# eso28599/resnmtf

Measured on AMD Instinct MI355X. Metric: multiplicative-update iters/sec (all views), higher is better.
Workload: dtype f32

## Files before the change

### resnmtf_amd/csrc/resnmtf_hip.hip

```cpp
#include <hip/hip_runtime.h>
#include <hip/hip_ext.h>

#include <algorithm>
#include <chrono>
#include <cmath>
#include <cstdlib>
#include <cstdio>
#include <cstring>
#include <random>
#include <string>
#include <thread>
#include <type_traits>
#include <vector>

#include "resnmtf_hip.h"
#include "resnmtf_kernels.hip.inc"
#include "resnmtf_sparse.hip.inc"
#include "resnmtf_jsd.hip.inc"
#include "resnmtf_group.hip.inc"
#include "resnmtf_bisil.hip.inc"
#include "resnmtf_split_tu.h"
#ifdef RESNMTF_SPLIT_TU
#define RESNMTF_EXTERN(NW, UNR, XG, MA) extern template __global__ void pass_kernel<1, NW, UNR, XG, MA, 0>(PassArgs, KKFArgs, KKSArgs);
RESNMTF_PASS_K16_LIST(RESNMTF_EXTERN)
#undef RESNMTF_EXTERN
#endif

namespace {

std::string g_create_error;

inline int round_up(int x, int a) { return (x + a - 1) / a * a; }
inline int ceil_div(int x, int a) { return (x + a - 1) / a; }

struct SharedMap {
  bool set = false;
  int count = -1;
  int* dev = nullptr;
  bool identity = false;
};

struct ViewState {
  int n = 0, m = 0, k = 0, KP = 16, NT = 1;
  bool owned = true, has_x = false, has_factors = false;
  int empty_rows = 0, empty_cols = 0;
  std::vector<unsigned char> empty_mask;
  unsigned char* ref_cl = nullptr;
  int ref_k = 0;
  int n_pad = 0, m_pad = 0;
  size_t ldx = 0, ldxt = 0;
  size_t x32_floats = 0, xt32_floats = 0;
  bool half = false, u16 = false;
  bool half_capable = false;
  double x_relerr = 0.0;
  _Float16 *X16 = nullptr, *Xt16 = nullptr;
  size_t ld16x = 0, ld16xt = 0, x16_halves = 0, xt16_halves = 0;
  float xscale = 1.f;
  float *X32 = nullptr, *Xt32 = nullptr;
  double* xnorm2 = nullptr;
  double *F = nullptr, *G = nullptr, *S = nullptr, *lambda = nullptr, *mu = nullptr;
  float *F32 = nullptr, *G32 = nullptr, *T32 = nullptr;
  unsigned short *Fk = nullptr, *Gk = nullptr;
  int nsplit_xg = 1, rps_xg = 64, nw_xg = 4, nsaux_xg = 1, rpsaux_xg = 64;
  int nsplit_xtf = 1, rps_xtf = 64, nw_xtf = 4, nsaux_xtf = 1, rpsaux_xtf = 64;
  int tw_xg = 8, tw_xtf = 8;
  float *Pxg = nullptr, *Pxtf = nullptr, *Paux_xg = nullptr, *Paux_xtf = nullptr;
  int *cnt_xg = nullptr, *cnt_xtf = nullptr;
  int* fuse_cnt = nullptr;
  int rpbF = 16, nblkF = 1, rpbG = 16, nblkG = 1;
  void* fblk = nullptr;
  size_t fblk_bytes = 0;
  float* Usum = nullptr;
  bool f_replica = false;
  void* gblk = nullptr; size_t gblk_bytes = 0;
  float* Tsum = nullptr;
  bool g_replica = false;
  double* sblk = nullptr;
  bool pp_xg = false, pp_xtf = false;
  int kk_mode = 0;
  double *partF = nullptr, *partG = nullptr;
  double *FtF = nullptr, *FtFS = nullptr, *cF = nullptr;
  double *Ma_F = nullptr, *Md_F = nullptr, *Ma_G = nullptr, *Md_G = nullptr;
  std::vector<SharedMap> row_map, col_map;
  UpdateArgs argF{}, argG{};
  KKFArgs argKF{};
  KKSArgs argKS{};
  PassArgs passXG{}, passXtF{};
  bool sparse = false;
  long long nnz_cap = 0, nnz = 0;
  long long *cp = nullptr, *rp = nullptr;
  int *ri = nullptr, *ci = nullptr;
  float *vcsc = nullptr, *vcsr = nullptr;
  int *blk_xg = nullptr, *blk_xtf = nullptr;
  int nblk_xg = 0, nblk_xtf = 0;
};

}

struct resnmtf_handle {
  int V = 0;
  std::vector<ViewState> views;
  resnmtf_options opt{};
  hipStream_t stream = nullptr;
  bool own_stream = false;
  std::vector<double> phi, xi, psi;
  SweepCtl* ctl = nullptr;
  double* err = nullptr;
// ... 101 lines not shown
auto pick_int(int x, F&& f) {
  if constexpr (sizeof...(Vs) == 0) return f(std::integral_constant<int, V0>{});
  else return x == V0 ? f(std::integral_constant<int, V0>{}) : pick_int<Vs...>(x, f);
}
template <class F>
auto pick_kp(int KP, F&& f) { return pick_int<16, 32, 48, 64>(KP, f); }
template <class F>
auto pick_bools(F&& f) { return f(); }
template <class F, class... Bs>
auto pick_bools(F&& f, bool b, Bs... bs) {
  return b ? pick_bools([&](auto... cs) { return f(std::true_type{}, cs...); }, bs...)
           : pick_bools([&](auto... cs) { return f(std::false_type{}, cs...); }, bs...);
}
constexpr int kKPs[] = {16, 32, 48, 64};
constexpr bool kBools[] = {false, true};

void free_view(ViewState& v) {
  if (v.fblk) { v.fblk = nullptr; v.Usum = nullptr; v.Ma_F = nullptr; v.Md_F = nullptr; v.lambda = nullptr; }
  if (v.gblk) { v.gblk = nullptr; v.Tsum = nullptr; v.Ma_G = nullptr; v.Md_G = nullptr; v.mu = nullptr; }
  v.sblk = nullptr;
  void* ptrs[] = {v.fuse_cnt, v.Fk, v.Gk, v.X16, v.Xt16, v.X32, v.Xt32, v.xnorm2, v.F, v.G, v.S, v.lambda, v.mu, v.F32, v.G32, v.T32, v.Pxg, v.Pxtf,
                  v.Paux_xg, v.Paux_xtf, v.cnt_xg, v.cnt_xtf, v.partF, v.partG, v.FtF, v.FtFS, v.cF, v.Ma_F, v.Md_F, v.Ma_G, v.Md_G, v.ref_cl,
                  v.cp, v.rp, v.ri, v.ci, v.vcsc, v.vcsr, v.blk_xg, v.blk_xtf};
  for (void* p : ptrs)
    if (p) (void)hipFree(p);
  for (auto& mp : v.row_map)
    if (mp.dev) (void)hipFree(mp.dev);
  for (auto& mp : v.col_map)
    if (mp.dev) (void)hipFree(mp.dev);
}

int check_view(resnmtf_handle* h, int v) {
  if (!h) return RESNMTF_ERR_INVALID;
  if (v < 0 || v >= h->V) return h->fail(RESNMTF_ERR_INVALID, "view index out of range");
  return RESNMTF_OK;
}

void to_row_major(const double* src, int rows, int cols, std::vector<double>& dst) {
  dst.resize((size_t)rows * cols);
  for (int j = 0; j < cols; ++j)
    for (int i = 0; i < rows; ++i) dst[(size_t)i * cols + j] = src[(size_t)j * rows + i];
}
void to_col_major(const std::vector<double>& src, int rows, int cols, double* dst) {
  for (int j = 0; j < cols; ++j)
    for (int i = 0; i < rows; ++i) dst[(size_t)j * rows + i] = src[(size_t)i * cols + j];
}

size_t update_smem_bytes(int KP) {
  const int UT = update_threads(KP), RG = UT / KP;
  const int P16 = (KP % 32 == 0) ? KP + 16 : KP + 32;
  return sizeof(double) * ((size_t)2 * KP * P16 + 2 * (size_t)RG * (KP + 2) + (size_t)RG * KP + 2 * UT + 2 * (size_t)RG * P16);
}
size_t kk_smem_bytes(int KP, int NW) { return sizeof(double) * ((size_t)4 * KP * KP + 3 * 64 * (size_t)NW); }
size_t pass_smem_bytes(int KP, int NW) {
  const size_t tile_form = std::max(sizeof(float) * (size_t)std::max(NW / 2, 1) * 64 * KP, kk_smem_bytes(KP, NW));
  return KP > 16 ? std::max(tile_form, wide_smem_bytes(KP / 16)) : tile_form;
}
constexpr int kMaxLds = 160 * 1024;

int max_pass_waves(int NT) { return NT <= 1 ? 16 : 8; }
int pass_blocks_per_cu(int NT, int nw) { return pass_min_blocks(NT, nw); }

using PassFn = void (*)(PassArgs, KKFArgs, KKSArgs);
using FusedFn = void (*)(PassArgs, KKFArgs, KKSArgs, UpdateArgs, FuseArgs);
using SpmmFn = void (*)(SpmmArgs, KKFArgs, KKSArgs);
template <int NVB> using WideFn = void (*)(WideChainArgs<NVB>);

struct PassK16Form { int nw, unroll; bool xg, mode_a; PassFn fn; };
const PassK16Form kPassK16[] = {
#define RESNMTF_FORM(NW, UNR, XG, MA) {NW, UNR, XG, MA, &pass_kernel<1, NW, UNR, XG, MA, 0>},
    RESNMTF_PASS_K16_LIST(RESNMTF_FORM)
#undef RESNMTF_FORM
};
PassFn select_pass(int NT, int nw, int unroll, bool xg, bool mode_a, bool wide) {
  if (NT <= 1) {
    for (const PassK16Form& f : kPassK16)
      if (!wide && f.nw == nw && f.unroll == unroll && f.xg == xg && f.mode_a == mode_a) return f.fn;
    return nullptr;
  }
  if (nw != 8 || unroll != 4) return nullptr;
  return pick_int<2, 3, 4>(NT, [&](auto nt) { return pick_bools([](auto x, auto m, auto w) {
    return &pass_kernel<decltype(nt)::value, 8, 4, decltype(x)::value, decltype(m)::value, (decltype(w)::value ? 3 : 0)>; }, xg, mode_a, wide); });
}
PassFn select_pass_half(int unroll, bool xg, bool u16) {
  return pick_int<2, 3, 6, 4>(unroll, [&](auto un) { return pick_bools([](auto x, auto u) { return &pass_half_kernel<decltype(un)::value, decltype(x)::value, decltype(u)::value>; }, xg, u16); });
}
FusedFn select_pass_fused(int unroll, bool xg, bool pre) {
  return pick_int<4, 8>(unroll, [&](auto un) { return pick_bools([](auto x, auto p) { return &pass_fused_kernel<decltype(un)::value, decltype(x)::value, decltype(p)::value>; }, xg, pre); });
}
SpmmFn select_spmm(int KP, bool xg) {
  return pick_kp(KP, [&](auto kp) { return pick_bools([](auto x) { return &spmm_kernel<decltype(kp)::value, decltype(x)::value>; }, xg); });
}
constexpr int kCoupleBuckets[] = {0, 4, 8, RESNMTF_MAX_COUPLE};
int couple_bucket(const UpdateArgs& a) { return !a.restricted ? 0 : a.n_couple <= 4 ? 4 : a.n_couple <= 8 ? 8 : RESNMTF_MAX_COUPLE; }
auto select_update(int KP, bool g, int bucket, bool emit) {
  return pick_kp(KP, [&](auto kp) { return pick_int<0, 4, 8, RESNMTF_MAX_COUPLE>(bucket, [&](auto nc) {
    return pick_bools([](auto G, auto E) { return &factor_update_kernel<decltype(kp)::value, decltype(G)::value, decltype(nc)::value, decltype(E)::value>; }, g, emit);
  }); });
}
template <int NVB>
auto select_f_chain(bool g, bool one_slab) { return g ? &f_chain_kernel<NVB, 1, true> : one_slab ? &f_chain_kernel<NVB, 1> : &f_chain_kernel<NVB, 4>; }
template <int NVB>
WideFn<NVB> select_wide_chain(int KP, bool g, bool sliced) {
  return pick_kp(KP, [&](auto kp) { return pick_bools([](auto G, auto S) -> WideFn<NVB> {
    constexpr int K = decltype(kp)::value;
    if constexpr (decltype(S)::value) return &wide_chain_kernel<K, decltype(G)::value, NVB, true>;
    else if constexpr (K >= 32) return &wide_chain_kernel<K, decltype(G)::value, NVB>;
    else return nullptr;
  }, g, sliced); });
}
template <int NVB>
auto select_slice_chain(int KP, bool g) {
  return pick_kp(KP, [&](auto kp) { return pick_bools([](auto G) { return &slice_chain_kernel<decltype(kp)::value, decltype(G)::value, NVB>; }, g); });
}
template <int NVB>
auto select_slice_products(int KP) { return pick_kp(KP, [](auto kp) { return &slice_products_kernel<decltype(kp)::value, NVB>; }); }
template <int NVB>
auto select_slice_walk(int KP) { return pick_kp(KP, [](auto kp) { return &slice_walk_kernel<decltype(kp)::value, NVB, 4>; }); }
auto select_slice_unpack(int KP) { return pick_kp(KP, [](auto kp) { return &slice_unpack_kernel<decltype(kp)::value>; }); }
constexpr int kSChainViews[] = {4, 8, RESNMTF_MAX_COUPLE + 1};
auto select_s_chain(int KP, int n_views) {
  const int nvb = n_views <= 4 ? 4 : n_views <= 8 ? 8 : RESNMTF_MAX_COUPLE + 1;
  return pick_kp(KP, [&](auto kp) { return pick_int<4, 8, RESNMTF_MAX_COUPLE + 1>(nvb, [](auto nv) { return &s_chain_kernel<decltype(kp)::value, decltype(nv)::value>; }); });
}

hipError_t set_all_attrs() {
  hipError_t e = hipSuccess;
  auto lds = [&](auto* fn, size_t bytes) {
    if (e == hipSuccess && fn) e = hipFuncSetAttribute(reinterpret_cast<const void*>(fn), hipFuncAttributeMaxDynamicSharedMemorySize, (int)bytes);
  };
  for (const PassK16Form& f : kPassK16) lds(f.fn, kMaxLds);
  for (bool xg : kBools)
    for (bool b : kBools) {
      for (int NT : {2, 3, 4}) { lds(select_pass(NT, 8, 4, xg, b, false), kMaxLds); lds(select_pass(NT, 8, 4, xg, b, true), kMaxLds); }
      for (int unroll : {4, 8}) lds(select_pass_fused(unroll, xg, b), kMaxLds);
    }
  for (int KP : kKPs) {
    for (bool g : kBools) {
      for (int bucket : kCoupleBuckets) { lds(select_update(KP, g, bucket, false), update_smem_bytes(KP)); lds(select_update(KP, g, bucket, true), update_smem_bytes(KP)); }
      for (bool sliced : kBools) { lds(select_wide_chain<4>(KP, g, sliced), wide_chain_smem_bytes(KP)); lds(select_wide_chain<8>(KP, g, sliced), wide_chain_smem_bytes(KP)); }
      lds(select_slice_chain<4>(KP, g), slice_chain_smem_bytes(KP, 4)); lds(select_slice_chain<8>(KP, g), slice_chain_smem_bytes(KP, 8));
      lds(select_spmm(KP, g), kk_smem_bytes(KP, 8));
    }
    for (int views : kSChainViews) lds(select_s_chain(KP, views), kMaxLds - 4096);
  }
  for (bool g : kBools)
    for (bool one_slab : kBools) { lds(select_f_chain<2>(g, one_slab), f_chain_smem_bytes<2>()); lds(select_f_chain<4>(g, one_slab), f_chain_smem_bytes<4>()); lds(select_f_chain<8>(g, one_slab), f_chain_smem_bytes<8>()); }
  return e;
}

SpmmArgs spmm_args(const ViewState& v, bool xg) {
  SpmmArgs a{};
  if (xg) { a.ptr = v.rp; a.idx = v.ci; a.val = v.vcsr; a.blk = v.blk_xg; a.nblk = v.nblk_xg; a.nsplit = v.nsplit_xg; a.B = v.G32; a.P = v.Pxg; a.cols_pad = v.n_pad; }
  else { a.ptr = v.cp; a.idx = v.ri; a.val = v.vcsc; a.blk = v.blk_xtf; a.nblk = v.nblk_xtf; a.nsplit = v.nsplit_xtf; a.B = v.F32; a.P = v.Pxtf; a.cols_pad = v.m_pad; }
  a.ldb = v.KP;
  return a;
}
dim3 spmm_grid(const SpmmArgs& a) { return dim3((a.kk_block0 ? 1 : 0) + ceil_div(a.nblk * a.nsplit, 8)); }
size_t spmm_smem(const SpmmArgs& a, int KP) { return a.kk_block0 && !a.no_kk ? kk_smem_bytes(KP, 8) : 0; }
void launch_spmm(resnmtf_handle* h, const SpmmArgs& a, int KP, bool xg, const KKFArgs& kf, const KKSArgs& ks) {
  launch(h, -1, select_spmm(KP, xg), spmm_grid(a), dim3(512), spmm_smem(a, KP), a, kf, ks);
}

struct PassLaunch {
  int image = 0;
  bool mode_a = true;
  bool fused = false;
  bool wide = false;
  bool xcd_order = false;
  bool short_last = false;
  bool pingpong = false;
  int waves = 8;
  int unroll = 0;
  int tiles_per_wg = 1;
  int lead_blocks = 1, main_blocks = 0;
  dim3 grid, block;
  size_t smem = 0;
  PassFn kern = nullptr;
  FusedFn kern_fused = nullptr;
  SpmmFn kern_spmm = nullptr;
};
PassLaunch resolve_pass(const resnmtf_handle* h, const ViewState& v, bool xg, bool fuse_update = false) {
  PassLaunch L;
  if (v.sparse) {
    SpmmArgs a = spmm_args(v, xg);
    a.kk_block0 = 1;
    L.image = 1;
    L.main_blocks = ceil_div(a.nblk * a.nsplit, 8);
    L.grid = spmm_grid(a); L.block = dim3(512);
    L.smem = spmm_smem(a, v.KP);
    L.kern_spmm = select_spmm(v.KP, xg);
    return L;
  }
  const int nw = xg ? v.nw_xg : v.nw_xtf, nsplit = xg ? v.nsplit_xg : v.nsplit_xtf, rps = xg ? v.rps_xg : v.rps_xtf;
  const int rows_pad = xg ? v.m_pad : v.n_pad, ntiles = (xg ? v.n_pad : v.m_pad) / 64;
  L.image = v.half ? (v.u16 ? 3 : 2) : 0;
  L.mode_a = v.kk_mode == 0;
  L.waves = nw;
  L.wide = v.NT >= 2 && h->opt.bf16_split != 2;
  L.xcd_order = L.wide && h->opt.xcd_order;
  L.short_last = nsplit > 1 && rows_pad - (nsplit - 1) * rps < rps;
  L.tiles_per_wg = L.wide ? (xg ? v.tw_xg : v.tw_xtf) : 1;
  L.main_blocks = ceil_div(ntiles, L.tiles_per_wg) * nsplit;
  L.lead_blocks = L.mode_a ? 1 : (xg ? 3 * v.nsaux_xg : 2 * v.nsaux_xtf);
  L.grid = dim3(L.lead_blocks + L.main_blocks); L.block = dim3(64 * nw);
  L.smem = std::min<size_t>(pass_smem_bytes(v.KP, nw) + (size_t)h->opt.pass_lds_pad_kb * 1024, kMaxLds);
  const bool pp = xg ? v.pp_xg : v.pp_xtf;
  if (fuse_update) {
    L.fused = true;
    L.pingpong = pp;
    L.unroll = pp ? 4 : 8;
    L.smem = std::min<size_t>(std::max(L.smem, update_smem_bytes(16)), kMaxLds);
    L.kern_fused = select_pass_fused(L.unroll, xg, h->opt.fuse_updates == 1);
  } else if (v.half) {
    const int hu = h->opt.half_unroll;
    L.unroll = (hu == 2 || hu == 3 || hu == 4 || hu == 6) ? hu : (v.u16 ? 2 : 4);
    L.kern = select_pass_half(L.unroll, xg, v.u16);
  } else {
    L.pingpong = v.NT == 1 && nw == 8 && pp;
    L.unroll = v.NT >= 2 ? 4 : (nw == 8 ? (pp ? 4 : RESNMTF_K16_UNROLL) : 8);
    L.kern = select_pass(v.NT, nw, L.unroll, xg, L.mode_a, L.wide);
  }
  return L;
}
bool can_fuse_update(const resnmtf_handle* h, const ViewState& v, int kind) {
  if (h->opt.fuse_updates == 0 || v.NT != 1 || !v.fuse_cnt) return false;
  const PassLaunch L = resolve_pass(h, v, kind != 0);
  if (L.image != 0 || !L.mode_a || L.waves != 8) return false;
  const UpdateArgs& u = kind == 0 ? v.argF : v.argG;
  const int nblk = kind == 0 ? v.nblkF : v.nblkG;
  return !u.restricted && nblk <= L.main_blocks && nblk <= h->n_cu;
}
void launch_pass(resnmtf_handle* h, const ViewState& v, bool xg, int mode, double tol, bool check_done, bool fuse_update = false) {
  const PassLaunch L = resolve_pass(h, v, xg, fuse_update);
  const int kind = xg ? RESNMTF_TIMED_XG : RESNMTF_TIMED_XTF;
  KKFArgs kf = v.argKF;
  KKSArgs ks = v.argKS;
  ks.mode = mode; ks.tol = tol;
  if (L.kern_spmm) {
    SpmmArgs a = spmm_args(v, xg);
    a.kk_block0 = 1; a.no_kk = 0; a.ctl = h->ctl; a.check_done = check_done ? 1 : 0;
    launch(h, kind, L.kern_spmm, L.grid, L.block, L.smem, a, kf, ks);
    return;
  }
  PassArgs a = xg ? v.passXG : v.passXtF;
  a.check_done = check_done ? 1 : 0;
  a.kk_block0 = L.mode_a ? 1 : 0;
  a.fuse_zero = (a.kk_block0 && v.fuse_cnt && !v.half) ? v.fuse_cnt + (xg ? 0 : 2) : nullptr;
  if (!a.kk_block0) { kf.part = nullptr; ks.part = nullptr; }
  a.xcd_n = 0;
  if (L.xcd_order) {
    const int n_map = L.short_last ? (a.nsplit - 1) * a.ntg : L.main_blocks;
    int cnt[8] = {0, 0, 0, 0, 0, 0, 0, 0};
    for (int x = 0; x < 8; ++x) a.xcd_first[x] = -1;
    for (int b = 0; b < n_map; ++b) {
      const int x = (L.lead_blocks + b) & 7;
      if (a.xcd_first[x] < 0) a.xcd_first[x] = L.lead_blocks + b;
      ++cnt[x];
    }
    int off = 0;
    for (int x = 0; x < 8; ++x) { a.xcd_off[x] = off; off += cnt[x]; if (a.xcd_first[x] < 0) a.xcd_first[x] = 0; }
    a.xcd_n = n_map;
  }
  if (L.fused) {
    UpdateArgs u = xg ? v.argG : v.argF;
    u.check_done = 0; u.gram_only = 0;
    FuseArgs fz{};
    fz.cnt_own = v.fuse_cnt + (xg ? 2 : 0);
    { static const int nap = std::getenv("RESNMTF_FUSE_NAP") ? std::atoi(std::getenv("RESNMTF_FUSE_NAP")) : 2; fz.nap = nap; }
    fz.n_upd = xg ? v.nblkG : v.nblkF; fz.err = h->fuse_err_dev;
    launch(h, kind, L.kern_fused, L.grid, L.block, L.smem, a, kf, ks, u, fz);
    return;
  }
  if (L.image >= 2) a.out_scale = v.u16 ? 1.f / v.xscale : 1.f / (v.xscale * RESNMTF_B16_SCALE);
  launch(h, kind, L.kern, L.grid, L.block, L.smem, a, kf, ks);
}

void launch_pass_plain(resnmtf_handle* h, PassArgs a, int NT, bool xg) {
  a.kk_block0 = 1; a.no_kk = 1; a.check_done = 0;
  const dim3 grid(1 + a.ntiles * a.nsplit), block(64 * 8);
  const size_t smem = std::min<size_t>(pass_smem_bytes(16 * NT, 8), kMaxLds);
  launch(h, -1, select_pass(NT, 8, NT <= 1 ? RESNMTF_K16_UNROLL : 4, xg, true, false), grid, block, smem, a, KKFArgs{}, KKSArgs{});
}

template <int NVB>
ChainArgs<NVB> narrow_chain(const ChainArgs<8>& c) {
  ChainArgs<NVB> a{};
  a.len = c.len; a.k = c.k; a.n_views = c.n_views; a.rows_per_block = c.rows_per_block;
  a.n_emit = c.n_emit; a.restricted = c.restricted; a.ctl = c.ctl; a.check_done = c.check_done; a.pstride = c.pstride;
  a.kpack32 = c.kpack32;
  for (int e = 0; e < 4; ++e) { a.W32e[e] = c.W32e[e]; a.parte[e] = c.parte[e]; a.T32e[e] = c.T32e[e]; }
  for (int v = 0; v < NVB; ++v) {
    a.emit_slot[v] = c.emit_slot[v];
    a.W[v] = c.W[v]; a.U[v] = c.U[v]; a.nsplit[v] = c.nsplit[v]; a.Ma[v] = c.Ma[v]; a.Md[v] = c.Md[v]; a.lm[v] = c.lm[v];
    a.sigma[v] = c.sigma[v]; a.n_other[v] = c.n_other[v]; a.cmask[v] = c.cmask[v];
    for (int w = 0; w < NVB; ++w) a.weight[v][w] = c.weight[v][w];
  }
  return a;
}

void launch_update(resnmtf_handle* h, const ViewState& v, int kind, bool check_done) {
  UpdateArgs a = kind == 0 ? v.argF : v.argG;
  a.check_done = check_done ? 1 : 0;
  a.gram_only = kind == 2 ? 1 : 0;
  if (kind == 2) { a.restricted = 0; a.n_couple = 0; }
  const int nblk = kind == 0 ? v.nblkF : v.nblkG;
  launch(h, -1, select_update(v.KP, kind != 0, couple_bucket(a), v.kk_mode == 0), dim3(nblk), dim3(update_threads(v.KP)), update_smem_bytes(v.KP), a);
}

template <int NVB>
WideChainArgs<NVB> narrow_wchain(const WideChainArgs<8>& c) {
  WideChainArgs<NVB> a{};
  a.len = c.len; a.k = c.k; a.n_views = c.n_views; a.ngroups = c.ngroups; a.own = c.own; a.n_self = c.n_self; a.O32 = c.O32; a.o32_stride = c.o32_stride;
  a.W32 = c.W32; a.Wk = c.Wk; a.T32 = c.T32; a.ld32 = c.ld32; a.ctl = c.ctl; a.check_done = c.check_done; a.restricted = c.restricted;
  for (int v = 0; v < NVB; ++v) {
    a.W[v] = c.W[v]; a.U[v] = c.U[v]; a.Ma[v] = c.Ma[v]; a.Md[v] = c.Md[v]; a.lm[v] = c.lm[v]; a.O32v[v] = c.O32v[v];
    a.sigma[v] = c.sigma[v]; a.n_other[v] = c.n_other[v]; a.cmask[v] = c.cmask[v];
    for (int w = 0; w < NVB; ++w) a.weight[v][w] = c.weight[v][w];
  }
  return a;
}
template <class F>
void for_wchain(const WideChainArgs<8>& c, F&& f) {
  if (c.n_views <= 4) f(std::integral_constant<int, 4>{}, narrow_wchain<4>(c));
  else f(std::integral_constant<int, 8>{}, c);
}
template <class F>
void for_chain(const ChainArgs<8>& c, int views, F&& f) {
  if (views <= 2) f(std::integral_constant<int, 2>{}, narrow_chain<2>(c));
  else if (views <= 4) f(std::integral_constant<int, 4>{}, narrow_chain<4>(c));
  else f(std::integral_constant<int, 8>{}, c);
}
// ... 3128 lines not shown
```

### resnmtf_amd/csrc/resnmtf_kernels.hip.inc

```

typedef float f32x4 __attribute__((ext_vector_type(4)));
typedef double f64x4 __attribute__((ext_vector_type(4)));
__host__ __device__ __forceinline__ size_t xidx(int r, int c, size_t ts) { return (size_t)(c >> 6) * ts + (size_t)r * 64 + (c & 63); }

#ifdef RESNMTF_STAMPS
__device__ unsigned long long* g_stamp_buf = nullptr;
__device__ int g_stamp_sel = 3;
#define STAMP_IF(bit, idx)                                                              \
  do {                                                                                  \
    if (g_stamp_buf && (g_stamp_sel & (bit)) && threadIdx.x == 0) g_stamp_buf[(size_t)blockIdx.x * 16 + (idx)] = wall_clock64(); \
  } while (0)
#define STAMP(idx) STAMP_IF(1, idx)
#define STAMP_U(idx) STAMP_IF(2, idx)
#else
#define STAMP(idx) do { } while (0)
#define STAMP_U(idx) do { } while (0)
#endif

struct SweepCtl {
  int sweep;
  int done;
  int stop_sweep;
  int pad;
  double prev_mean;
// ... 207 lines not shown
  }
  }
  if (sq_err) {
#pragma unroll
    for (int off = 32; off > 0; off >>= 1) e2 += __shfl_xor(e2, off);
    if ((threadIdx.x & 63) == 0) red[threadIdx.x >> 6] = e2;
    __syncthreads();
    if (threadIdx.x == 0) atomicAdd(sq_err, red[0] + red[1] + red[2] + red[3]);
  }
}

#define RESNMTF_MAX_AUX 3
struct PassArgs {
  const float* A; int lda; int ntiles;
  size_t tile_stride;
  const _Float16* A16; size_t tile_stride16;
  float out_scale;
  const float* B; int ldb;
  const unsigned short* Bk;
  int tw, ntg;
  float* P;
  int cols_pad;
  int rows_pad;
  int rows_per_split; int nsplit;
  const float* aux[RESNMTF_MAX_AUX];
  int naux;
  float* Paux;
  int rows_per_split_aux; int nsplit_aux;
  int* aux_cnt;
  int kk_block0;
  int no_kk;
  const SweepCtl* ctl; int check_done;
  int* fuse_zero;
  int xcd_n; int xcd_first[8]; int xcd_off[8];
};
__device__ __forceinline__ int xcd_order(const PassArgs& a, int b , int gi ) {
  if (b >= a.xcd_n) return b;
  const int x = gi & 7;
  return a.xcd_off[x] + ((gi - a.xcd_first[x]) >> 3);
}

template <int NT, int NW>
__device__ __forceinline__ void pass_epilogue(f32x4 (&acc)[4][NT], float* red , float* __restrict__ out ) {
  constexpr int KP = 16 * NT;
  const int lane = threadIdx.x & 63, wave = threadIdx.x >> 6;
  const int p = lane & 15, q = lane >> 4;
#pragma unroll
  for (int s = NW / 2; s >= 1; s >>= 1) {
    if (wave >= s && wave < 2 * s) {
      float* slot = red + (size_t)(wave - s) * 64 * KP;
#pragma unroll
      for (int jj = 0; jj < 4; ++jj)
#pragma unroll
        for (int nt = 0; nt < NT; ++nt)
#pragma unroll
          for (int t = 0; t < 4; ++t) slot[((jj * NT + nt) * 4 + t) * 64 + lane] = acc[jj][nt][t];
    }
    __syncthreads();
    if (wave < s) {
      const float* slot = red + (size_t)wave * 64 * KP;
#pragma unroll
      for (int jj = 0; jj < 4; ++jj)
#pragma unroll
        for (int nt = 0; nt < NT; ++nt)
#pragma unroll
          for (int t = 0; t < 4; ++t) acc[jj][nt][t] += slot[((jj * NT + nt) * 4 + t) * 64 + lane];
    }
    __syncthreads();
  }
  if (wave == 0) {
#pragma unroll
    for (int jj = 0; jj < 4; ++jj)
#pragma unroll
      for (int nt = 0; nt < NT; ++nt)
#pragma unroll
        for (int t = 0; t < 4; ++t)
          red[(16 * q + 4 * t + jj) * KP + 16 * nt + p] = acc[jj][nt][t];
  }
  __syncthreads();
  for (int e = threadIdx.x * 4; e < 64 * KP; e += 256 * NW)
    *reinterpret_cast<f32x4*>(out + e) = *reinterpret_cast<const f32x4*>(&red[e]);
}

template <int NW, int UNROLL>
__device__ __forceinline__ bool pass_prefetch_a(const float* __restrict__ A, int lda, int r_begin, int r_end, f32x4 (&av)[UNROLL]) {
  const int lane = threadIdx.x & 63, wave = threadIdx.x >> 6;
  const int nsteps = (r_end - r_begin) / (4 * NW);
  const bool usable = UNROLL == 4 ? nsteps >= 2 * UNROLL : nsteps >= UNROLL;
  const float* a_ptr = A + (size_t)(r_begin + 4 * wave + (lane >> 4)) * lda + 4 * (lane & 15);
  const size_t a_step = (size_t)4 * NW * lda;
#pragma unroll
  for (int u = 0; u < UNROLL; ++u) av[u] = *reinterpret_cast<const f32x4*>(a_ptr + (size_t)(usable ? u : 0) * a_step);
  return usable;
}
template <int NT, int NW, int UNROLL, bool PRE = false>
__device__ __forceinline__ void pass_body(const float* __restrict__ A, int lda, const float* __restrict__ B, int ldb,
                                          int r_begin, int r_end, float* red ,
                                          float* __restrict__ out , const f32x4* pre_av = nullptr) {
  constexpr int KP = 16 * NT;
  const int lane = threadIdx.x & 63, wave = threadIdx.x >> 6;
  const int p = lane & 15, q = lane >> 4;
  const int nsteps = (r_end - r_begin) / (4 * NW);

  f32x4 acc[4][NT];
#pragma unroll
  for (int jj = 0; jj < 4; ++jj)
#pragma unroll
    for (int nt = 0; nt < NT; ++nt) acc[jj][nt] = (f32x4){0.f, 0.f, 0.f, 0.f};

  const int row0 = r_begin + 4 * wave + q;
  const float* b_ptr = B + (size_t)row0 * ldb + p * NT;
  const size_t b_step = (size_t)4 * NW * ldb;
  if (A != nullptr) {
    const float* a_ptr = A + (size_t)row0 * lda + 4 * p;
    const size_t a_step = (size_t)4 * NW * lda;
    auto load_full = [&](int i, f32x4 (&av)[UNROLL], float (&bv)[UNROLL][NT]) {
#pragma unroll
      for (int u = 0; u < UNROLL; ++u) {
        if (NT >= 2) av[u] = __builtin_nontemporal_load(reinterpret_cast<const f32x4*>(a_ptr + (size_t)(i + u) * a_step));
        else av[u] = *reinterpret_cast<const f32x4*>(a_ptr + (size_t)(i + u) * a_step);
        load_b<NT>(b_ptr + (size_t)(i + u) * b_step, bv[u]);
      }
    };
    auto load_masked = [&](int i, f32x4 (&av)[UNROLL], float (&bv)[UNROLL][NT]) {
#pragma unroll
      for (int u = 0; u < UNROLL; ++u) {
        const bool in = i + u < nsteps;
        const int st = in ? i + u : nsteps - 1;
        const f32x4 a = *reinterpret_cast<const f32x4*>(a_ptr + (size_t)st * a_step);
        av[u] = in ? a : (f32x4){0.f, 0.f, 0.f, 0.f};
        float b[NT];
        load_b<NT>(b_ptr + (size_t)st * b_step, b);
#pragma unroll
        for (int nt = 0; nt < NT; ++nt) bv[u][nt] = in ? b[nt] : 0.f;
      }
    };
    auto load_first = [&](f32x4 (&av)[UNROLL], float (&bv)[UNROLL][NT]) {
      if (PRE) {
#pragma unroll
        for (int u = 0; u < UNROLL; ++u) { av[u] = pre_av[u]; load_b<NT>(b_ptr + (size_t)u * b_step, bv[u]); }
      } else {
        load_full(0, av, bv);
      }
    };
    auto mma_trip = [&](const f32x4 (&av)[UNROLL], const float (&bv)[UNROLL][NT]) {
#pragma unroll
      for (int u = 0; u < UNROLL; ++u)
#pragma unroll
        for (int jj = 0; jj < 4; ++jj)
#pragma unroll
          for (int nt = 0; nt < NT; ++nt)
            acc[jj][nt] = __builtin_amdgcn_mfma_f32_16x16x4f32(av[u][jj], bv[u][nt], acc[jj][nt], 0, 0, 0);
    };
    int done = 0;
    if (NT >= 2 || UNROLL == 4) {
      const int ndouble = nsteps / (2 * UNROLL);
      if (ndouble > 0) {
        f32x4 a0[UNROLL], a1[UNROLL];
        float b0[UNROLL][NT], b1[UNROLL][NT];
        load_first(a0, b0);
        for (int d = 0; d < ndouble; ++d) {
          const int i = d * 2 * UNROLL;
          load_full(i + UNROLL, a1, b1);
          mma_trip(a0, b0);
          if (d + 1 < ndouble) load_full(i + 2 * UNROLL, a0, b0);
          mma_trip(a1, b1);
        }
      }
      done = ndouble * 2 * UNROLL;
    } else {
      const int nfull = nsteps / UNROLL;
      if (PRE && nfull > 0) {
        f32x4 av[UNROLL];
        float bv[UNROLL][NT];
        load_first(av, bv);
        mma_trip(av, bv);
      }
      for (int t = (PRE && nfull > 0) ? 1 : 0; t < nfull; ++t) {
        f32x4 av[UNROLL];
        float bv[UNROLL][NT];
        load_full(t * UNROLL, av, bv);
        mma_trip(av, bv);
      }
      done = nfull * UNROLL;
    }
    for (int i = done; i < nsteps; i += UNROLL) {
      f32x4 av[UNROLL];
      float bv[UNROLL][NT];
      load_masked(i, av, bv);
      mma_trip(av, bv);
    }
  } else {
    for (int i = 0; i < nsteps; ++i) {
      float b[NT];
      load_b<NT>(b_ptr + (size_t)i * b_step, b);
#pragma unroll
      for (int nt = 0; nt < NT; ++nt) acc[0][nt] = __builtin_amdgcn_mfma_f32_16x16x4f32(1.0f, b[nt], acc[0][nt], 0, 0, 0);
    }
#pragma unroll
    for (int nt = 0; nt < NT; ++nt) { acc[1][nt] = acc[0][nt]; acc[2][nt] = acc[0][nt]; acc[3][nt] = acc[0][nt]; }
  }

  pass_epilogue<NT, NW>(acc, red, out);
}


typedef __bf16 bf16x8_t __attribute__((ext_vector_type(8)));
typedef unsigned int u32x4_t __attribute__((ext_vector_type(4)));
__host__ __device__ __forceinline__ size_t bk_index(int r, int i, int NT, int piece) {
  return ((((size_t)(r >> 5) * NT + (i >> 4)) * 3 + piece) * 64 + (r & 3) * 16 + (i & 15)) * 8 + ((r & 31) >> 2);
}
typedef float f32x2_t __attribute__((ext_vector_type(2)));
typedef __bf16 bf16x2_t __attribute__((ext_vector_type(2)));
__device__ __forceinline__ unsigned int pk_bf16(float a, float b) {
  const f32x2_t v = {a, b};
  return __builtin_bit_cast(unsigned int, __builtin_convertvector(v, bf16x2_t));
}
__device__ __forceinline__ void bk_store(unsigned short* __restrict__ Bk, int r, int i, int NT, float x) {
  const unsigned int h = pk_bf16(x, 0.f) & 0xFFFFu;
  const float r1 = x - __uint_as_float(h << 16);
  const unsigned int m = pk_bf16(r1, 0.f) & 0xFFFFu;
  const float r2 = r1 - __uint_as_float(m << 16);
  const size_t at = bk_index(r, i, NT, 0);
  Bk[at] = (unsigned short)h;
  Bk[at + 512] = (unsigned short)m;
  Bk[at + 1024] = (unsigned short)(pk_bf16(r2, 0.f) & 0xFFFFu);
}
__host__ __device__ constexpr int wide_buf_frags(int NT, int RW) { return (NT * 3 * 64 * RW + 511) / 512 * 512; }
__host__ __device__ constexpr size_t wide_smem_bytes(int NT) {
  return (size_t)2 * wide_buf_frags(NT, 2) * 16 > (size_t)4 * 64 * 16 * NT * 4 ? (size_t)2 * wide_buf_frags(NT, 2) * 16 : (size_t)4 * 64 * 16 * NT * 4;
}

template <int NT, int RW>
__device__ __forceinline__ void pass_body_wide(const float* __restrict__ A, size_t tile_stride, int ntiles, int tile0,
                                               const unsigned short* __restrict__ Bk, int r_begin, int r_end,
                                               u32x4_t* __restrict__ lds, float* __restrict__ out_split ) {
  constexpr int KP = 16 * NT, NQ = NT * 3 * 64;
  constexpr int TW = 8 / RW, BUF = wide_buf_frags(NT, RW), NB = BUF / 512, nq = NQ * RW;
  const int lane = threadIdx.x & 63, wave = __builtin_amdgcn_readfirstlane(threadIdx.x >> 6), p = lane & 15, q = lane >> 4;
  const int tl = wave % TW, rg = wave / TW;
  const int tile = tile0 + tl;
  const bool valid = tile < ntiles;
  constexpr int trip_rows = 32 * RW;
  const int ntrip = (r_end - r_begin) / trip_rows;
  f32x4 acc[4][NT];
#pragma unroll
  for (int jj = 0; jj < 4; ++jj)
#pragma unroll
    for (int nt = 0; nt < NT; ++nt) acc[jj][nt] = (f32x4){0.f, 0.f, 0.f, 0.f};
  const float* a_ptr = A + (size_t)(valid ? tile : ntiles - 1) * tile_stride + (size_t)(r_begin + 32 * rg + q) * 64 + 4 * p;
  constexpr size_t a_trip = (size_t)trip_rows * 64;
  const u32x4_t* bg = reinterpret_cast<const u32x4_t*>(Bk) + (size_t)(r_begin >> 5) * NQ;
  u32x4_t* ldsB = lds;
  int bidx[NB];
#pragma unroll
  for (int e = 0; e < NB; ++e) bidx[e] = min((int)threadIdx.x + 512 * e, nq - 1);
  auto load_a = [&](int t, f32x4 (&av)[8]) {
#pragma unroll
    for (int u = 0; u < 8; ++u) av[u] = __builtin_nontemporal_load(reinterpret_cast<const f32x4*>(a_ptr + (size_t)t * a_trip + (size_t)u * 256));
  };
  auto load_bg = [&](int t, u32x4_t (&g)[NB]) {
#pragma unroll
    for (int e = 0; e < NB; ++e) g[e] = bg[(size_t)t * nq + bidx[e]];
  };
  auto store_b = [&](int buf, const u32x4_t (&g)[NB]) {
#pragma unroll
    for (int e = 0; e < NB; ++e) ldsB[buf * BUF + threadIdx.x + 512 * e] = g[e];
  };
  auto compute = [&](const f32x4 (&av)[8], int buf) {
    u32x4_t bq[NT][3];
#pragma unroll
    for (int nt = 0; nt < NT; ++nt)
#pragma unroll
      for (int pc = 0; pc < 3; ++pc) bq[nt][pc] = ldsB[buf * BUF + rg * NQ + (nt * 3 + pc) * 64 + lane];
#pragma unroll
    for (int jj = 0; jj < 4; ++jj) {
      u32x4_t ah, am, al;
#pragma unroll
      for (int d = 0; d < 4; ++d) {
        const float x0 = av[2 * d][jj], x1 = av[2 * d + 1][jj];
        const unsigned int ph = pk_bf16(x0, x1);
        const float r0 = x0 - __uint_as_float(ph << 16), r1 = x1 - __uint_as_float(ph & 0xFFFF0000u);
        const unsigned int pm = pk_bf16(r0, r1);
        const float s0 = r0 - __uint_as_float(pm << 16), s1 = r1 - __uint_as_float(pm & 0xFFFF0000u);
        ah[d] = ph; am[d] = pm; al[d] = pk_bf16(s0, s1);
      }
// ... 1846 lines not shown
      return;
    }
    const int tile = b % a.ntiles, split = b / a.ntiles;
    const int r_begin = split * a.rows_per_split;
      pass_body<NT, NW, UNROLL>(a.A + (size_t)tile * a.tile_stride, a.lda, a.B, a.ldb, r_begin, min(r_begin + a.rows_per_split, a.rows_pad), red,
                                a.P + ((size_t)split * a.cols_pad + (size_t)tile * 64) * KP);
    STAMP(SB + 1);
    return;
  }
  const int naux_blocks = a.naux * a.nsplit_aux;
  if ((int)blockIdx.x >= naux_blocks) {
    const int b = blockIdx.x - naux_blocks;
    if (SPLIT >= 2 && NW == 8) {
      const int bx = xcd_order(a, b, (int)blockIdx.x);
      const int tg = bx % a.ntg, split = bx / a.ntg;
      const int r_begin = split * a.rows_per_split;
      if (a.tw == 8)
        pass_body_wide<NT, 1>(a.A, a.tile_stride, a.ntiles, tg * 8, a.Bk, r_begin, min(r_begin + a.rows_per_split, a.rows_pad),
                              reinterpret_cast<u32x4_t*>(smem_d), a.P + (size_t)split * a.cols_pad * KP);
      else
        pass_body_wide<NT, 2>(a.A, a.tile_stride, a.ntiles, tg * 4, a.Bk, r_begin, min(r_begin + a.rows_per_split, a.rows_pad),
                              reinterpret_cast<u32x4_t*>(smem_d), a.P + (size_t)split * a.cols_pad * KP);
      STAMP(SB + 1);
      return;
    }
    const int tile = b % a.ntiles, split = b / a.ntiles;
    const int r_begin = split * a.rows_per_split;
      pass_body<NT, NW, UNROLL>(a.A + (size_t)tile * a.tile_stride, a.lda, a.B, a.ldb, r_begin, min(r_begin + a.rows_per_split, a.rows_pad), red,
                                a.P + ((size_t)split * a.cols_pad + (size_t)tile * 64) * KP);
    STAMP(SB + 1);
    return;
  }
  const int kind = blockIdx.x / a.nsplit_aux, split = blockIdx.x % a.nsplit_aux;
  const int r_begin = split * a.rows_per_split_aux;
  constexpr bool PREFETCH = (KP * KP <= 2 * 64 * NW);
  KKSPre<KP, 64 * NW> pre_s; KKFPre<KP, 64 * NW> pre_f;
  if (PREFETCH) { if (IS_XG) kk_s_prefetch<KP, 64 * NW>(ks, pre_s); else kk_f_prefetch<KP, 64 * NW>(kf, pre_f); }
  pass_body<NT, NW, UNROLL>(a.aux[kind], 64, a.B, a.ldb, r_begin, min(r_begin + a.rows_per_split_aux, a.rows_pad), red,
                            a.Paux + ((size_t)kind * a.nsplit_aux + split) * 64 * KP);
  STAMP(SB + 1);
  asm volatile("s_waitcnt vmcnt(0)" ::: "memory");
  __syncthreads();
  volatile int* ticket_slot = reinterpret_cast<volatile int*>(red);
  if (threadIdx.x == 0) {
    __builtin_amdgcn_fence(__ATOMIC_RELEASE, "agent");
    asm volatile("s_waitcnt vmcnt(0)" ::: "memory");
    *ticket_slot = __hip_atomic_fetch_add(a.aux_cnt, 1, __ATOMIC_RELAXED, __HIP_MEMORY_SCOPE_AGENT);
  }
  __syncthreads();
  const int ticket = *ticket_slot;
  STAMP(SB + 2);
  if (ticket != naux_blocks - 1) return;
  if (threadIdx.x == 0) {
    __builtin_amdgcn_fence(__ATOMIC_ACQUIRE, "agent");
    asm volatile("s_waitcnt vmcnt(0)" ::: "memory");
    __hip_atomic_store(a.aux_cnt, 0, __ATOMIC_RELAXED, __HIP_MEMORY_SCOPE_AGENT);
  }
  __syncthreads();
  STAMP(SB + 3);
  if (IS_XG) { if (!PREFETCH) kk_s_prefetch<KP, 64 * NW>(ks, pre_s); kk_s_body<KP, 64 * NW, false>(ks, pre_s, a.Paux, a.nsplit_aux, smem_d); }
  else { if (!PREFETCH) kk_f_prefetch<KP, 64 * NW>(kf, pre_f); kk_f_body<KP, 64 * NW, false>(kf, pre_f, a.Paux, a.nsplit_aux, smem_d); }
  STAMP(SB + 4);
}

template <int UNROLL, bool IS_XG, bool U16>
__global__ __launch_bounds__(512, 4) void pass_half_kernel(PassArgs a, KKFArgs kf, KKSArgs ks) {
  constexpr int KP = 16, NW = 8;
  if (a.check_done && a.ctl->done) return;
  extern __shared__ __attribute__((aligned(16))) double smem_d[];
  float* red = reinterpret_cast<float*>(smem_d);
  if (blockIdx.x == 0) {
    if (a.no_kk) return;
    if (IS_XG) { KKSPre<KP, 64 * NW> pre; kk_s_prefetch<KP, 64 * NW>(ks, pre); kk_s_body<KP, 64 * NW, true>(ks, pre, a.Paux, a.nsplit_aux, smem_d); }
    else { KKFPre<KP, 64 * NW> pre; kk_f_prefetch<KP, 64 * NW>(kf, pre); kk_f_body<KP, 64 * NW, true>(kf, pre, a.Paux, a.nsplit_aux, smem_d); }
    return;
  }
  const int b = blockIdx.x - 1;
  const int tile = b % a.ntiles, split = b / a.ntiles;
  const int r_begin = split * a.rows_per_split;
  pass_body_half<NW, UNROLL, U16>(a.A16 + (size_t)tile * a.tile_stride16, a.B, r_begin, min(r_begin + a.rows_per_split, a.rows_pad),
                             a.out_scale, red, a.P + ((size_t)split * a.cols_pad + (size_t)tile * 64) * KP);
}

struct FuseArgs {
  int* cnt_own;
  int n_upd;
  int* err;
  int nap;
};
template <int UNROLL, bool IS_XG, bool PRE>
__global__ __launch_bounds__(512, 4) void pass_fused_kernel(PassArgs a, KKFArgs kf, KKSArgs ks, UpdateArgs u, FuseArgs fz) {
  constexpr int KP = 16, NT = 1, NW = 8;
  constexpr int SB = IS_XG ? 0 : 8;
  (void)SB;
  if (a.check_done && a.ctl->done) return;
  extern __shared__ __attribute__((aligned(16))) double smem_d[];
  float* red = reinterpret_cast<float*>(smem_d);
  STAMP(SB + 0);
  const int b = (int)blockIdx.x - 1;
  KKSPre<KP, 64 * NW> pre_s; KKFPre<KP, 64 * NW> pre_f;
  if (b < 0) {
    if (a.fuse_zero && threadIdx.x < 2) __hip_atomic_store(a.fuse_zero + threadIdx.x, 0, __ATOMIC_RELAXED, __HIP_MEMORY_SCOPE_AGENT);
    if (!a.no_kk) {
      if (IS_XG) kk_s_prefetch<KP, 64 * NW>(ks, pre_s); else kk_f_prefetch<KP, 64 * NW>(kf, pre_f);
    }
  } else if (b < fz.n_upd) {
    factor_update_body<KP, IS_XG, 0, true>(u, b, smem_d);
    asm volatile("s_waitcnt vmcnt(0)" ::: "memory");
    __syncthreads();
    STAMP(SB + 5);
    if (threadIdx.x == 0) {
      __builtin_amdgcn_fence(__ATOMIC_RELEASE, "agent");
      asm volatile("s_waitcnt vmcnt(0)" ::: "memory");
      if (__hip_atomic_fetch_add(fz.cnt_own, 1, __ATOMIC_RELAXED, __HIP_MEMORY_SCOPE_AGENT) == fz.n_upd - 1)
        __hip_atomic_store(fz.cnt_own + 1, 1, __ATOMIC_RELAXED, __HIP_MEMORY_SCOPE_AGENT);
    }
  }
  f32x4 pre_av[UNROLL];
  const int tile = b < 0 ? 0 : b % a.ntiles, split = b < 0 ? 0 : b / a.ntiles;
  const int r_begin = split * a.rows_per_split, r_end = min(r_begin + a.rows_per_split, a.rows_pad);
  bool pre_ok = false;
  if (PRE && b >= 0) pre_ok = pass_prefetch_a<NW, UNROLL>(a.A + (size_t)tile * a.tile_stride, a.lda, r_begin, r_end, pre_av);
  if (threadIdx.x == 0) {
    int spins = 0;
    while (__hip_atomic_load(fz.cnt_own + 1, __ATOMIC_RELAXED, __HIP_MEMORY_SCOPE_AGENT) == 0) {
      for (int z = 0; z < fz.nap; ++z) __builtin_amdgcn_s_sleep(8);
      if (++spins > (1 << 19)) { __hip_atomic_store(fz.err, 1, __ATOMIC_RELAXED, __HIP_MEMORY_SCOPE_AGENT); break; }
    }
#ifdef RESNMTF_FUSE_ACQUIRE
    __builtin_amdgcn_fence(__ATOMIC_ACQUIRE, "agent");
    asm volatile("s_waitcnt vmcnt(0)" ::: "memory");
#endif
  }
  asm volatile("" ::: "memory");
  __syncthreads();
  STAMP(SB + 6);
  if (b < 0) {
    if (a.no_kk) return;
    if (IS_XG) kk_s_body<KP, 64 * NW, true>(ks, pre_s, a.Paux, a.nsplit_aux, smem_d);
    else kk_f_body<KP, 64 * NW, true>(kf, pre_f, a.Paux, a.nsplit_aux, smem_d);
    STAMP(SB + 4);
    return;
  }
  float* out = a.P + ((size_t)split * a.cols_pad + (size_t)tile * 64) * KP;
  if (PRE && pre_ok) pass_body<NT, NW, UNROLL, true>(a.A + (size_t)tile * a.tile_stride, a.lda, a.B, a.ldb, r_begin, r_end, red, out, pre_av);
  else pass_body<NT, NW, UNROLL>(a.A + (size_t)tile * a.tile_stride, a.lda, a.B, a.ldb, r_begin, r_end, red, out);
  STAMP(SB + 1);
}

struct SlicePackArgs {
  const float* P; int nsplit; int rows_pad;
  int KP, NT;
  int rows_per_slice, n_slices;
  char* out; size_t chunk_bytes;
  char* outv[8];
  const double* tail[2]; int tail_count;
  double* tailv[8];
  float* T32; int ld32;
  const SweepCtl* ctl; int check_done;
};
static __global__ __launch_bounds__(256) void slice_pack_kernel(SlicePackArgs a) {
  if (a.check_done && a.ctl->done) return;
  const int qpr = a.KP / 4;
  const size_t quads_all = (size_t)a.n_slices * a.rows_per_slice * qpr;
  const size_t slab_quads = (size_t)a.rows_pad * qpr;
  for (size_t idx = (size_t)blockIdx.x * 256 + threadIdx.x; idx < quads_all; idx += (size_t)gridDim.x * 256) {
// ... 311 lines not shown
```

### resnmtf_amd/csrc/resnmtf_pass_k16.hip

```cpp
#include <hip/hip_runtime.h>
#include <hip/hip_ext.h>

#include <algorithm>
#include <cmath>
#include <cstdlib>
#include <cstdio>
#include <cstring>
#include <type_traits>

#include "resnmtf_hip.h"
#include "resnmtf_kernels.hip.inc"
#include "resnmtf_split_tu.h"

#define RESNMTF_INSTANTIATE(NW, UNR, XG, MA) template __global__ void pass_kernel<1, NW, UNR, XG, MA, 0>(PassArgs, KKFArgs, KKSArgs);
RESNMTF_PASS_K16_LIST(RESNMTF_INSTANTIATE)
#undef RESNMTF_INSTANTIATE
```

### resnmtf_amd/csrc/resnmtf_split_tu.h

```cpp
#ifndef RESNMTF_SPLIT_TU_H
#define RESNMTF_SPLIT_TU_H
#ifndef RESNMTF_K16_UNROLL
#define RESNMTF_K16_UNROLL 8
#endif
#define RESNMTF_PASS_K16_LIST(X)                                                              \
  X(4, 8, true, true) X(4, 8, true, false) X(4, 8, false, true) X(4, 8, false, false)         \
  X(8, 4, true, true) X(8, 4, true, false) X(8, 4, false, true) X(8, 4, false, false)         \
  X(8, RESNMTF_K16_UNROLL, true, true) X(8, RESNMTF_K16_UNROLL, true, false) X(8, RESNMTF_K16_UNROLL, false, true) X(8, RESNMTF_K16_UNROLL, false, false) \
  X(16, 8, true, true) X(16, 8, true, false) X(16, 8, false, true) X(16, 8, false, false)
#endif
```

Baseline: 22870.

## Add paired-tile pass kernel sharing B loads across two column tiles

Adds a pass_pair_kernel in which each workgroup computes two adjacent 64-column tiles, loading each B value once and reusing it for both tiles' MFMA accumulations. A flat LDS epilogue reduces the per-wave partial sums for both tiles. The K16 mode-A path with 8 waves and no ping-pong now dispatches to this kernel, halving the number of main blocks. It removes redundant B traffic and per-block overhead, at the cost of twice the accumulator registers, more LDS for the reduction, fewer workgroups, and a fixed unroll of 4 in place of 8.

```diff
diff --git a/resnmtf_amd/csrc/resnmtf_hip.hip b/resnmtf_amd/csrc/resnmtf_hip.hip
--- a/resnmtf_amd/csrc/resnmtf_hip.hip
+++ b/resnmtf_amd/csrc/resnmtf_hip.hip
@@ -23,6 +23,9 @@
 #ifdef RESNMTF_SPLIT_TU
 #define RESNMTF_EXTERN(NW, UNR, XG, MA) extern template __global__ void pass_kernel<1, NW, UNR, XG, MA, 0>(PassArgs, KKFArgs, KKSArgs);
 RESNMTF_PASS_K16_LIST(RESNMTF_EXTERN)
+#undef RESNMTF_EXTERN
+#define RESNMTF_EXTERN(UNR, XG) extern template __global__ void pass_pair_kernel<UNR, XG>(PassArgs, KKFArgs, KKSArgs);
+RESNMTF_PASS_PAIR_LIST(RESNMTF_EXTERN)
 #undef RESNMTF_EXTERN
 #endif
 
@@ -290,6 +293,17 @@
   return pick_int<2, 3, 4>(NT, [&](auto nt) { return pick_bools([](auto x, auto m, auto w) {
     return &pass_kernel<decltype(nt)::value, 8, 4, decltype(x)::value, decltype(m)::value, (decltype(w)::value ? 3 : 0)>; }, xg, mode_a, wide); });
 }
+struct PassPairForm { int unroll; bool xg; PassFn fn; };
+const PassPairForm kPassPair[] = {
+#define RESNMTF_FORM(UNR, XG) {UNR, XG, &pass_pair_kernel<UNR, XG>},
+    RESNMTF_PASS_PAIR_LIST(RESNMTF_FORM)
+#undef RESNMTF_FORM
+};
+PassFn select_pass_pair(int unroll, bool xg) {
+  for (const PassPairForm& f : kPassPair)
+    if (f.unroll == unroll && f.xg == xg) return f.fn;
+  return nullptr;
+}
 PassFn select_pass_half(int unroll, bool xg, bool u16) {
   return pick_int<2, 3, 6, 4>(unroll, [&](auto un) { return pick_bools([](auto x, auto u) { return &pass_half_kernel<decltype(un)::value, decltype(x)::value, decltype(u)::value>; }, xg, u16); });
 }
@@ -338,6 +352,7 @@
     if (e == hipSuccess && fn) e = hipFuncSetAttribute(reinterpret_cast<const void*>(fn), hipFuncAttributeMaxDynamicSharedMemorySize, (int)bytes);
   };
   for (const PassK16Form& f : kPassK16) lds(f.fn, kMaxLds);
+  for (const PassPairForm& f : kPassPair) lds(f.fn, kMaxLds);
   for (bool xg : kBools)
     for (bool b : kBools) {
       for (int NT : {2, 3, 4}) { lds(select_pass(NT, 8, 4, xg, b, false), kMaxLds); lds(select_pass(NT, 8, 4, xg, b, true), kMaxLds); }
@@ -378,6 +393,7 @@
   bool xcd_order = false;
   bool short_last = false;
   bool pingpong = false;
+  bool pair = false;
   int waves = 8;
   int unroll = 0;
   int tiles_per_wg = 1;
@@ -424,6 +440,14 @@
     const int hu = h->opt.half_unroll;
     L.unroll = (hu == 2 || hu == 3 || hu == 4 || hu == 6) ? hu : (v.u16 ? 2 : 4);
     L.kern = select_pass_half(L.unroll, xg, v.u16);
+  } else if (v.NT == 1 && L.mode_a && nw == 8 && !pp && ntiles >= 2) {
+    L.pair = true;
+    L.tiles_per_wg = 2;
+    L.main_blocks = ceil_div(ntiles, 2) * nsplit;
+    L.grid = dim3(L.lead_blocks + L.main_blocks);
+    L.unroll = RESNMTF_PAIR_UNROLL;
+    L.smem = std::min<size_t>(std::max(pass_pair_red_bytes(), kk_smem_bytes(v.KP, nw)) + (size_t)h->opt.pass_lds_pad_kb * 1024, kMaxLds);
+    L.kern = select_pass_pair(L.unroll, xg);
   } else {
     L.pingpong = v.NT == 1 && nw == 8 && pp;
     L.unroll = v.NT >= 2 ? 4 : (nw == 8 ? (pp ? 4 : RESNMTF_K16_UNROLL) : 8);
@@ -433,7 +457,7 @@
 }
 bool can_fuse_update(const resnmtf_handle* h, const ViewState& v, int kind) {
   if (h->opt.fuse_updates == 0 || v.NT != 1 || !v.fuse_cnt) return false;
-  const PassLaunch L = resolve_pass(h, v, kind != 0);
+  const PassLaunch L = resolve_pass(h, v, kind != 0, true);
   if (L.image != 0 || !L.mode_a || L.waves != 8) return false;
   const UpdateArgs& u = kind == 0 ? v.argF : v.argG;
   const int nblk = kind == 0 ? v.nblkF : v.nblkG;
@@ -456,6 +480,7 @@
   a.kk_block0 = L.mode_a ? 1 : 0;
   a.fuse_zero = (a.kk_block0 && v.fuse_cnt && !v.half) ? v.fuse_cnt + (xg ? 0 : 2) : nullptr;
   if (!a.kk_block0) { kf.part = nullptr; ks.part = nullptr; }
+  if (L.pair) { a.tw = 2; a.ntg = ceil_div(a.ntiles, 2); }
   a.xcd_n = 0;
   if (L.xcd_order) {
     const int n_map = L.short_last ? (a.nsplit - 1) * a.ntg : L.main_blocks;
diff --git a/resnmtf_amd/csrc/resnmtf_kernels.hip.inc b/resnmtf_amd/csrc/resnmtf_kernels.hip.inc
--- a/resnmtf_amd/csrc/resnmtf_kernels.hip.inc
+++ b/resnmtf_amd/csrc/resnmtf_kernels.hip.inc
@@ -313,6 +313,42 @@
     *reinterpret_cast<f32x4*>(out + e) = *reinterpret_cast<const f32x4*>(&red[e]);
 }
 
+template <int NT, int NW, int TW>
+__device__ __forceinline__ void pass_epilogue_flat(f32x4 (&acc)[TW][4][NT], float* red , float* (&out)[TW] ) {
+  constexpr int KP = 16 * NT;
+  static_assert(KP % NW == 0, "whole accumulator registers per thread");
+  const int lane = threadIdx.x & 63, wave = threadIdx.x >> 6;
+#pragma unroll
+  for (int tw = 0; tw < TW; ++tw) {
+    float* slot = red + (size_t)(tw * NW + wave) * 64 * KP;
+#pragma unroll
+    for (int jj = 0; jj < 4; ++jj)
+#pragma unroll
+      for (int nt = 0; nt < NT; ++nt)
+#pragma unroll
+        for (int t = 0; t < 4; ++t) slot[((jj * NT + nt) * 4 + t) * 64 + lane] = acc[tw][jj][nt][t];
+  }
+  __syncthreads();
+#pragma unroll
+  for (int tw = 0; tw < TW; ++tw) {
+    if (out[tw] == nullptr) continue;
+    const float* base = red + (size_t)tw * NW * 64 * KP;
+#pragma unroll
+    for (int j = 0; j < 64 * KP / (64 * NW); ++j) {
+      const int reg = wave + NW * j;
+      float v[NW];
+#pragma unroll
+      for (int w = 0; w < NW; ++w) v[w] = base[(size_t)w * 64 * KP + reg * 64 + lane];
+#pragma unroll
+      for (int s = NW / 2; s >= 1; s >>= 1)
+#pragma unroll
+        for (int w = 0; w < s; ++w) v[w] += v[w + s];
+      const int t = reg & 3, nt = (reg >> 2) % NT, jj = (reg >> 2) / NT;
+      out[tw][(16 * (lane >> 4) + 4 * t + jj) * KP + 16 * nt + (lane & 15)] = v[0];
+    }
+  }
+}
+
 template <int NW, int UNROLL>
 __device__ __forceinline__ bool pass_prefetch_a(const float* __restrict__ A, int lda, int r_begin, int r_end, f32x4 (&av)[UNROLL]) {
   const int lane = threadIdx.x & 63, wave = threadIdx.x >> 6;
@@ -433,6 +469,71 @@
   }
 
   pass_epilogue<NT, NW>(acc, red, out);
+}
+
+template <int NW, int UNROLL, int TW>
+__device__ __forceinline__ void pass_body_tiles(const float* __restrict__ A, size_t tile_stride, const float* __restrict__ B, int ldb,
+                                                int r_begin, int r_end, float* red , float* (&out)[TW] ) {
+  const int lane = threadIdx.x & 63, wave = threadIdx.x >> 6;
+  const int p = lane & 15, q = lane >> 4;
+  const int nsteps = (r_end - r_begin) / (4 * NW);
+
+  f32x4 acc[TW][4][1];
+#pragma unroll
+  for (int tw = 0; tw < TW; ++tw)
+#pragma unroll
+    for (int jj = 0; jj < 4; ++jj) acc[tw][jj][0] = (f32x4){0.f, 0.f, 0.f, 0.f};
+
+  const int row0 = r_begin + 4 * wave + q;
+  const float* b_ptr = B + (size_t)row0 * ldb + p;
+  const size_t b_step = (size_t)4 * NW * ldb;
+  const float* a_ptr = A + (size_t)row0 * 64 + 4 * p;
+  const size_t a_step = (size_t)4 * NW * 64;
+  auto load_full = [&](int i, f32x4 (&av)[UNROLL][TW], float (&bv)[UNROLL]) {
+#pragma unroll
+    for (int u = 0; u < UNROLL; ++u) {
+#pragma unroll
+      for (int tw = 0; tw < TW; ++tw) av[u][tw] = *reinterpret_cast<const f32x4*>(a_ptr + (size_t)tw * tile_stride + (size_t)(i + u) * a_step);
+      bv[u] = b_ptr[(size_t)(i + u) * b_step];
+    }
+  };
+  auto load_masked = [&](int i, f32x4 (&av)[UNROLL][TW], float (&bv)[UNROLL]) {
+#pragma unroll
+    for (int u = 0; u < UNROLL; ++u) {
+      const bool in = i + u < nsteps;
+      const int st = in ? i + u : nsteps - 1;
+#pragma unroll
+      for (int tw = 0; tw < TW; ++tw) {
+        const f32x4 a = *reinterpret_cast<const f32x4*>(a_ptr + (size_t)tw * tile_stride + (size_t)st * a_step);
+        av[u][tw] = in ? a : (f32x4){0.f, 0.f, 0.f, 0.f};
+      }
+      const float b = b_ptr[(size_t)st * b_step];
+      bv[u] = in ? b : 0.f;
+    }
+  };
+  auto mma_trip = [&](const f32x4 (&av)[UNROLL][TW], const float (&bv)[UNROLL]) {
+#pragma unroll
+    for (int u = 0; u < UNROLL; ++u)
+#pragma unroll
+      for (int tw = 0; tw < TW; ++tw)
+#pragma unroll
+        for (int jj = 0; jj < 4; ++jj)
+          acc[tw][jj][0] = __builtin_amdgcn_mfma_f32_16x16x4f32(av[u][tw][jj], bv[u], acc[tw][jj][0], 0, 0, 0);
+  };
+  const int nfull = nsteps / UNROLL;
+  for (int t = 0; t < nfull; ++t) {
+    f32x4 av[UNROLL][TW];
+    float bv[UNROLL];
+    load_full(t * UNROLL, av, bv);
+    mma_trip(av, bv);
+  }
+  for (int i = nfull * UNROLL; i < nsteps; i += UNROLL) {
+    f32x4 av[UNROLL][TW];
+    float bv[UNROLL];
+    load_masked(i, av, bv);
+    mma_trip(av, bv);
+  }
+  pass_epilogue_flat<1, NW, TW>(acc, red, out);
 }
 
 
@@ -2445,6 +2546,35 @@
                              a.out_scale, red, a.P + ((size_t)split * a.cols_pad + (size_t)tile * 64) * KP);
 }
 
+constexpr size_t pass_pair_red_bytes() { return sizeof(float) * 2 * 8 * 64 * 16; }
+template <int UNROLL, bool IS_XG>
+__global__ __launch_bounds__(512, 4) void pass_pair_kernel(PassArgs a, KKFArgs kf, KKSArgs ks) {
+  constexpr int KP = 16, NW = 8;
+  constexpr int SB = IS_XG ? 0 : 8;
+  (void)SB;
+  if (a.check_done && a.ctl->done) return;
+  extern __shared__ __attribute__((aligned(16))) double smem_d[];
+  STAMP(SB + 0);
+  if (blockIdx.x == 0) {
+    if (a.fuse_zero && threadIdx.x < 2) __hip_atomic_store(a.fuse_zero + threadIdx.x, 0, __ATOMIC_RELAXED, __HIP_MEMORY_SCOPE_AGENT);
+    if (a.no_kk) return;
+    if (IS_XG) { KKSPre<KP, 64 * NW> pre; kk_s_prefetch<KP, 64 * NW>(ks, pre); kk_s_body<KP, 64 * NW, true>(ks, pre, a.Paux, a.nsplit_aux, smem_d); }
+    else { KKFPre<KP, 64 * NW> pre; kk_f_prefetch<KP, 64 * NW>(kf, pre); kk_f_body<KP, 64 * NW, true>(kf, pre, a.Paux, a.nsplit_aux, smem_d); }
+    STAMP(SB + 4);
+    return;
+  }
+  const int b = blockIdx.x - 1;
+  const int tile = (b % a.ntg) * 2, split = b / a.ntg;
+  const int r_begin = split * a.rows_per_split;
+  const bool both = tile + 1 < a.ntiles;
+  float* outs[2];
+  outs[0] = a.P + ((size_t)split * a.cols_pad + (size_t)tile * 64) * KP;
+  outs[1] = both ? outs[0] + 64 * KP : nullptr;
+  pass_body_tiles<NW, UNROLL, 2>(a.A + (size_t)tile * a.tile_stride, both ? a.tile_stride : 0, a.B, a.ldb, r_begin,
+                                 min(r_begin + a.rows_per_split, a.rows_pad), reinterpret_cast<float*>(smem_d), outs);
+  STAMP(SB + 1);
+}
+
 struct FuseArgs {
   int* cnt_own;
   int n_upd;
diff --git a/resnmtf_amd/csrc/resnmtf_pass_k16.hip b/resnmtf_amd/csrc/resnmtf_pass_k16.hip
--- a/resnmtf_amd/csrc/resnmtf_pass_k16.hip
+++ b/resnmtf_amd/csrc/resnmtf_pass_k16.hip
@@ -15,3 +15,6 @@
 #define RESNMTF_INSTANTIATE(NW, UNR, XG, MA) template __global__ void pass_kernel<1, NW, UNR, XG, MA, 0>(PassArgs, KKFArgs, KKSArgs);
 RESNMTF_PASS_K16_LIST(RESNMTF_INSTANTIATE)
 #undef RESNMTF_INSTANTIATE
+#define RESNMTF_INSTANTIATE(UNR, XG) template __global__ void pass_pair_kernel<UNR, XG>(PassArgs, KKFArgs, KKSArgs);
+RESNMTF_PASS_PAIR_LIST(RESNMTF_INSTANTIATE)
+#undef RESNMTF_INSTANTIATE
diff --git a/resnmtf_amd/csrc/resnmtf_split_tu.h b/resnmtf_amd/csrc/resnmtf_split_tu.h
--- a/resnmtf_amd/csrc/resnmtf_split_tu.h
+++ b/resnmtf_amd/csrc/resnmtf_split_tu.h
@@ -3,6 +3,10 @@
 #ifndef RESNMTF_K16_UNROLL
 #define RESNMTF_K16_UNROLL 8
 #endif
+#ifndef RESNMTF_PAIR_UNROLL
+#define RESNMTF_PAIR_UNROLL 4
+#endif
+#define RESNMTF_PASS_PAIR_LIST(X) X(RESNMTF_PAIR_UNROLL, true) X(RESNMTF_PAIR_UNROLL, false)
 #define RESNMTF_PASS_K16_LIST(X)                                                              \
   X(4, 8, true, true) X(4, 8, true, false) X(4, 8, false, true) X(4, 8, false, false)         \
   X(8, 4, true, true) X(8, 4, true, false) X(8, 4, false, true) X(8, 4, false, false)         \
```

Measured after the change: 21940. 0.959x the previous value.
